# luanfujun/Langevin-MCMC

Measured on AMD Instinct MI355X. Metric: MALA chain-steps/sec, torus scene, higher is better.
Workload: dtype f32

## Files before the change

### langevin-mcmc_amd/csrc/device/kernels.h

```cpp
#pragma once
#include <hip/hip_runtime.h>

#include "dchain.h"
#include "dstep_params.h"

namespace lmcd {
struct H2Arrays;
struct MalaPipe;
struct H2Bins;
struct H2MCParam;
}

void LaunchSeedRng(int n, long long firstSeed, uint64_t *state, uint32_t *tab, hipStream_t s);
void LaunchLowerBoundProbe(int n, const float *cdf, int nq, const float *u, int *out, hipStream_t s);
void LaunchRngProbe(int nSeeds, const unsigned long long *seeds, int mode, int n, float mean, float stddev, uint32_t *tabScratch, uint32_t *out, hipStream_t s);
void LaunchPluginGrad(int c, int l, const float *in, float *out, int wantGrad, hipStream_t s);
void LaunchPluginHess(int c, int l, const float *in, float *stage , float *out, hipStream_t s);
void LaunchCacheProbe(const lmcd::DCache *cache, int dim, int n, const float *u, int *row, const float *query, const int *cl, float *pdf, hipStream_t s);
void LaunchTransProbe(int n, int mode, const float *x, const float *y, float *o, hipStream_t s);
void LaunchStreamProbe(long long nWords, const float *in, float *out, hipStream_t s);
void LaunchAddInto(float *dst, const float *src, size_t n, hipStream_t s);
void LaunchAddIntoF64(double *dst, const double *src, size_t n, hipStream_t s);
void LaunchAddIntoI64(long long *dst, const long long *src, size_t n, hipStream_t s);
void LaunchFilmFixedToFloat(const long long *fx, float *rgb, size_t n, hipStream_t s);
// ... 22 lines not shown
                     uint32_t *tabScratch, float *contribScratch, const uint64_t *seedCkState, const uint32_t *seedCkTicks, float *initPath, float *initContrib,
                     float *initScoreSum, hipStream_t s);
void LaunchDirect(const lmcd::DScene &S, const lmcd::Film &film, int directSpp, int minDepth, int maxDepth, int bvhDepth, bool waveKernel, uint32_t *tabScratch,
                  hipStream_t s);
void LaunchBidirMC(const lmcd::DScene &S, const lmcd::Film &film, int nThreads, int samplesPerThread, uint32_t *tabScratch, float *contribScratch, hipStream_t s);
void LaunchMC(const lmcd::DScene &S, const lmcd::Film &film, bool bidirectional, int spp, int minDepth, int maxDepth, long long streamBegin, long long streamEnd,
              uint32_t *tabScratch, unsigned long long *counters, hipStream_t s);
long long MCThreads(const lmcd::DScene &S, long long streamBegin, long long streamEnd);
void LaunchMCFixedToFloat(const long long *fx, float *rgb, size_t n, int spp, hipStream_t s);
void LaunchSetupChains(const lmcd::ChainArrays &A, int chainBegin, long long perChain, long long chainsNeedExtra, hipStream_t s);
void LaunchFirstKind(const lmcd::DScene &S, const lmcd::DCache *cache, const lmcd::ChainArrays &A, const lmcd::StepParams &P, hipStream_t s);
void LaunchStepLarge(const lmcd::DScene &S, const lmcd::DCache *cache, const lmcd::ChainArrays &A, const lmcd::Film &film, const lmcd::StepParams &P,
                     const int *list, const int *listCount, const lmcd::NextLists &next, float *gradBuf, int gradStride, bool glossy, int gridBlocks, int bvhStackNeed, int blockThreads, hipStream_t s);
void LaunchStepLargeMux(const lmcd::DScene &S, const lmcd::DCache *cache, const lmcd::ChainArrays &A, const lmcd::Film &film, const lmcd::StepParams &P,
                     const int *list, const int *listCount, const lmcd::NextLists &next, float *gradBuf, int gradStride, bool glossy, int gridBlocks, int bvhStackNeed, int blockThreads, hipStream_t s);
void LaunchStepLargeCache(const lmcd::DScene &S, const lmcd::DCache *cache, const lmcd::ChainArrays &A, const lmcd::Film &film, const lmcd::StepParams &P,
                     const int *list, const int *listCount, const lmcd::NextLists &next, float *gradBuf, int gradStride, bool glossy, int gridBlocks, int bvhStackNeed, int blockThreads, hipStream_t s);
void LaunchStepSmallGrad(const lmcd::DScene &S, const lmcd::DCache *cache, const lmcd::ChainArrays &A, const lmcd::Film &film, const lmcd::StepParams &P,
                         const int *list, const int *listCount, const lmcd::NextLists &next, float *gradBuf, int gradStride, bool glossy, int gridBlocks, hipStream_t s);
void LaunchStepSmallLeanGrad(const lmcd::DScene &S, const lmcd::DCache *cache, const lmcd::ChainArrays &A, const lmcd::Film &film, const lmcd::StepParams &P, const int *list,
                             const int *listCount, const lmcd::NextLists &next, float *gradBuf, int gradStride, bool glossy, int gridBlocks, int blockThreads, int bvhStackNeed,
                             hipStream_t s);
void LaunchStepSmallPlain(const lmcd::DScene &S, const lmcd::DCache *cache, const lmcd::ChainArrays &A, const lmcd::Film &film, const lmcd::StepParams &P,
                          const int *list, const int *listCount, const lmcd::NextLists &next, int bvhDepth, bool glossy, int gridBlocks, int blockThreads,
                          bool profile, hipStream_t s);
void LaunchStepResident(const lmcd::DScene &S, const lmcd::DCache *cache, const lmcd::ChainArrays &A, const lmcd::Film &film, const lmcd::StepParams &P, int maxSteps,
                        int lanes, unsigned long long *guard, bool glossy, int mux, int bvhStackNeed, hipStream_t s);
void LaunchH2Begin(const lmcd::DScene &S, const lmcd::ChainArrays &A, const lmcd::StepParams &P, const lmcd::H2Arrays &H, const int *list, const int *listCount, int gridBlocks,
                   hipStream_t s);
void LaunchH2Perturb(const lmcd::DScene &S, const lmcd::ChainArrays &A, const lmcd::StepParams &P, const lmcd::H2Arrays &H, const int *list, const int *listCount,
                     int bvhStackNeed, int gridBlocks, hipStream_t s);
void LaunchH2Finish(const lmcd::DScene &S, const lmcd::DCache *cache, const lmcd::ChainArrays &A, const lmcd::Film &film, const lmcd::StepParams &P, const lmcd::H2Arrays &H,
                    const int *list, const int *listCount, int gridBlocks, hipStream_t s);
void LaunchH2Hess(const float *rec, const lmcd::H2Bins &bins, int N, const float *scene38 , float *hout, int gridBlocks, hipStream_t s);
void LaunchH2Gauss(const lmcd::H2Bins &bins, int N, const float *hout, const lmcd::H2MCParam &param, int expFlags, const int *chainFlags, int stage, float *gaussBuf,
                   const float *offsetSoA, float *px, int gridBlocks, hipStream_t s);
void LaunchH2Sample(const int *list, const int *listCount, int N, const int *chainFlags, const unsigned char *stepKind, const float *curContrib, const float *gaussBuf,
                    float sigma, float *offsetSoA, float *py, int gridBlocks, hipStream_t s);
void LaunchMalaBegin(const lmcd::DScene &S, const lmcd::DCache *cache, const lmcd::ChainArrays &A, const lmcd::StepParams &P, const lmcd::MalaPipe &M, const int *list,
                     const int *listCount, int gridBlocks, hipStream_t s);
void LaunchMalaMid(const lmcd::DScene &S, const lmcd::DCache *cache, const lmcd::ChainArrays &A, const lmcd::StepParams &P, const lmcd::MalaPipe &M, const int *list,
                   const int *listCount, int bvhStackNeed, bool glossy, int gridBlocks, hipStream_t s);
void LaunchMalaFinish(const lmcd::DScene &S, const lmcd::DCache *cache, const lmcd::ChainArrays &A, const lmcd::Film &film, const lmcd::StepParams &P, const lmcd::MalaPipe &M,
                      const int *list, const int *listCount, int gridBlocks, hipStream_t s);
void LaunchMalaGrad(const float *rec, const lmcd::H2Bins &bins, int N, const float *scene38 , float *gout, int gridBlocks, hipStream_t s);
void LaunchHessBatch(int c, int l, int n, const float *primarySoA, const float *scene, const float *vertSoA, float *logLum, float *gradSoA, float *hessSoA,
                     hipStream_t s);
// ... 41 lines not shown
```

### langevin-mcmc_amd/csrc/device/step_kernel.h

```cpp
#pragma once
#include "dstep.h"
#include "kernels.h"

namespace lmcd {

__device__ __forceinline__ void BlockReduceStats(const StepStats &st, unsigned long long *counters, double *weightSum, int *sh) {
    int *sInt = sh;
    float &sW = *reinterpret_cast<float *>(sh + 8);
    __syncthreads();
    if (threadIdx.x == 0) {
        for (int k = 0; k < 8; k++) sInt[k] = 0;
        sW = 0.f;
    }
    __syncthreads();
    int v[8] = {st.steps, st.large, st.accepted, st.gradCalls, st.cacheQueries, st.cacheHits, st.resets, st.lean};
    float w = st.wsum;
    for (int off = 32; off > 0; off >>= 1) {
        for (int k = 0; k < 8; k++) v[k] += __shfl_down(v[k], off);
        w += __shfl_down(w, off);
    }
    if ((threadIdx.x & 63) == 0) {
        for (int k = 0; k < 8; k++)
            if (v[k]) atomicAdd(&sInt[k], v[k]);
        atomicAdd(&sW, w);
    }
    __syncthreads();
    if (threadIdx.x == 0) {
        for (int k = 0; k < 8; k++)
            if (sInt[k]) atomicAdd(&counters[k], (unsigned long long)sInt[k]);
        if (sW != 0.f) atomicAdd(weightSum, (double)sW);
    }
}

#ifndef LMC_STEP_WAVES
#define LMC_STEP_WAVES 2
#endif
#ifndef LMC_STEP_WAVES_GLOSSY_LARGE
#define LMC_STEP_WAVES_GLOSSY_LARGE 3
#endif
template <class FILM, bool WITH_LARGE, bool WITH_SMALL, bool WITH_GRAD, bool GLOSSY, bool LDS_STACK = false, int MUX = 0, bool QUANT = false>
__global__ void __launch_bounds__(256, (GLOSSY && WITH_LARGE && !WITH_SMALL && LDS_STACK) ? LMC_STEP_WAVES_GLOSSY_LARGE : LMC_STEP_WAVES) k_step(DScene S, const DCache *cache, ChainArrays A, FILM film, StepParams P, const int *list, const int *listCount,
                                              NextLists next, float *gradBuf, int gradStride) {
    if ((int)(blockIdx.x * blockDim.x) >= *listCount) return;
    LMC_RNG_JUMP_INIT();
    LMC_MAT_LDS_INIT(S);
    extern __shared__ int ldsStack[];
    StepStats st;
    const int total = *listCount;
    const int tid = blockIdx.x * blockDim.x + threadIdx.x;
    for (int j = tid; j < total; j += gridDim.x * blockDim.x) {
        const int i = list[j];
        Rng rng = LoadChainRng(A, P.chainBegin, S.opt.seedOffset, i);
        GradWork gw{gradBuf, (size_t)gradStride, (size_t)tid};
        const int kind = WITH_LARGE ? KIND_LARGE : KIND_SMALL;
        if constexpr (LDS_STACK) {
            LdsStackT<GLOSSY, QUANT> stk{ldsStack + threadIdx.x, (int)blockDim.x, 0};
            StepChain<WITH_LARGE, WITH_SMALL, WITH_GRAD, MUX>(S, *cache, A, film, P, i, kind, rng, gw, st, stk);
        } else {
            LocalStackT<GLOSSY> stk;
            StepChain<WITH_LARGE, WITH_SMALL, WITH_GRAD, MUX>(S, *cache, A, film, P, i, kind, rng, gw, st, stk);
        }
        QueueNext(S, *cache, A, P, i, rng);
        StoreChainRng(A, i, rng);
    }
    __shared__ int sStats[9];
// ... 5 lines not shown
```

### langevin-mcmc_amd/csrc/device/step_large.hip

```cpp
#ifndef LMC_NO_RNG_JUMP_LDS
#define LMC_RNG_JUMP_LDS
#endif
#include "step_kernel.h"

using namespace lmcd;

template <class FILM>
static void LaunchStepLargeT(const DScene &S, const DCache *cache, const ChainArrays &A, const FILM &film, const StepParams &P, const int *list, const int *listCount,
                     const NextLists &next, float *gradBuf, int gradStride, bool glossy, int gridBlocks, int bvhStackNeed, int blockThreads, hipStream_t s) {
    RequireJumpLdsBlock(blockThreads);
    if (bvhStackNeed <= BVH_LDS_STACK) {
        const int blocks = gridBlocks * (256 / blockThreads);
        const size_t ldsBytes = (size_t)blockThreads * ((bvhStackNeed + 7) / 8 * 8) * sizeof(int);
        const bool quant = S.qnodes != nullptr;
        if (glossy && quant) hipLaunchKernelGGL((k_step<FILM, true, false, false, true, true, 0, true>), dim3(blocks), dim3(blockThreads), ldsBytes, s, S, cache, A, film, P, list, listCount, next, gradBuf, gradStride);
        else if (glossy) hipLaunchKernelGGL((k_step<FILM, true, false, false, true, true>), dim3(blocks), dim3(blockThreads), ldsBytes, s, S, cache, A, film, P, list, listCount, next, gradBuf, gradStride);
        else if (quant) hipLaunchKernelGGL((k_step<FILM, true, false, false, false, true, 0, true>), dim3(blocks), dim3(blockThreads), ldsBytes, s, S, cache, A, film, P, list, listCount, next, gradBuf, gradStride);
        else
            hipLaunchKernelGGL((k_step<FILM, true, false, false, false, true>), dim3(blocks), dim3(blockThreads), ldsBytes, s, S, cache, A, film, P, list, listCount, next, gradBuf, gradStride);
        return;
    }
    if (glossy) hipLaunchKernelGGL((k_step<FILM, true, false, false, true>), dim3(gridBlocks), dim3(256), 0, s, S, cache, A, film, P, list, listCount, next, gradBuf, gradStride);
    else
        hipLaunchKernelGGL((k_step<FILM, true, false, false, false>), dim3(gridBlocks), dim3(256), 0, s, S, cache, A, film, P, list, listCount, next, gradBuf, gradStride);
}
void LaunchStepLarge(const DScene &S, const DCache *cache, const ChainArrays &A, const Film &film, const StepParams &P, const int *list, const int *listCount,
                     const NextLists &next, float *gradBuf, int gradStride, bool glossy, int gridBlocks, int bvhStackNeed, int blockThreads, hipStream_t s) {
    DispatchFilm(film, [&](const auto &f) { LaunchStepLargeT(S, cache, A, f, P, list, listCount, next, gradBuf, gradStride, glossy, gridBlocks, bvhStackNeed, blockThreads, s); });
}
```

### langevin-mcmc_amd/csrc/device/step_large_cache.hip

```cpp
#ifndef LMC_NO_RNG_JUMP_LDS
#define LMC_RNG_JUMP_LDS
#endif
#include "step_kernel.h"

using namespace lmcd;

template <class FILM>
static void LaunchStepLargeCacheT(const DScene &S, const DCache *cache, const ChainArrays &A, const FILM &film, const StepParams &P, const int *list, const int *listCount,
                     const NextLists &next, float *gradBuf, int gradStride, bool glossy, int gridBlocks, int bvhStackNeed, int blockThreads, hipStream_t s) {
    RequireJumpLdsBlock(blockThreads);
    if (bvhStackNeed <= BVH_LDS_STACK) {
        const int blocks = gridBlocks * (256 / blockThreads);
        const size_t ldsBytes = (size_t)blockThreads * ((bvhStackNeed + 7) / 8 * 8) * sizeof(int);
        if (glossy) hipLaunchKernelGGL((k_step<FILM, true, false, false, true, true, 2>), dim3(blocks), dim3(blockThreads), ldsBytes, s, S, cache, A, film, P, list, listCount, next, gradBuf, gradStride);
        else
            hipLaunchKernelGGL((k_step<FILM, true, false, false, false, true, 2>), dim3(blocks), dim3(blockThreads), ldsBytes, s, S, cache, A, film, P, list, listCount, next, gradBuf, gradStride);
        return;
    }
    if (glossy) hipLaunchKernelGGL((k_step<FILM, true, false, false, true, false, 2>), dim3(gridBlocks), dim3(256), 0, s, S, cache, A, film, P, list, listCount, next, gradBuf, gradStride);
    else
        hipLaunchKernelGGL((k_step<FILM, true, false, false, false, false, 2>), dim3(gridBlocks), dim3(256), 0, s, S, cache, A, film, P, list, listCount, next, gradBuf, gradStride);
}
void LaunchStepLargeCache(const DScene &S, const DCache *cache, const ChainArrays &A, const Film &film, const StepParams &P, const int *list, const int *listCount,
                     const NextLists &next, float *gradBuf, int gradStride, bool glossy, int gridBlocks, int bvhStackNeed, int blockThreads, hipStream_t s) {
    DispatchFilm(film, [&](const auto &f) { LaunchStepLargeCacheT(S, cache, A, f, P, list, listCount, next, gradBuf, gradStride, glossy, gridBlocks, bvhStackNeed, blockThreads, s); });
}

__global__ void k_cache_probe(const DCache *cache, int dim, int n, const float *u, int *row, const float *query, const int *cl, float *pdf) {
    const DCacheDim &D = cache->d[dim];
    for (int i = blockIdx.x * blockDim.x + threadIdx.x; i < n; i += gridDim.x * blockDim.x) {
        row[i] = CacheSampleRow(D, u[i]);
        float q[MAXPSS];
        for (int k = 0; k < dim; k++) q[k] = query[(size_t)i * dim + k];
        pdf[i] = EvalPdfCache(D, dim, q, cl[2 * i], cl[2 * i + 1]);
    }
}
void LaunchCacheProbe(const DCache *cache, int dim, int n, const float *u, int *row, const float *query, const int *cl, float *pdf, hipStream_t s) {
    hipLaunchKernelGGL(k_cache_probe, dim3((n + 63) / 64), dim3(64), 0, s, cache, dim, n, u, row, query, cl, pdf);
}
```

### langevin-mcmc_amd/csrc/device/step_large_mux.hip

```cpp
#ifndef LMC_NO_RNG_JUMP_LDS
#define LMC_RNG_JUMP_LDS
#endif
#include "step_kernel.h"

using namespace lmcd;

template <class FILM>
static void LaunchStepLargeMuxT(const DScene &S, const DCache *cache, const ChainArrays &A, const FILM &film, const StepParams &P, const int *list, const int *listCount,
                     const NextLists &next, float *gradBuf, int gradStride, bool glossy, int gridBlocks, int bvhStackNeed, int blockThreads, hipStream_t s) {
    RequireJumpLdsBlock(blockThreads);
    if (bvhStackNeed <= BVH_LDS_STACK) {
        const int blocks = gridBlocks * (256 / blockThreads);
        const size_t ldsBytes = (size_t)blockThreads * ((bvhStackNeed + 7) / 8 * 8) * sizeof(int);
        if (glossy) hipLaunchKernelGGL((k_step<FILM, true, false, false, true, true, 1>), dim3(blocks), dim3(blockThreads), ldsBytes, s, S, cache, A, film, P, list, listCount, next, gradBuf, gradStride);
        else
            hipLaunchKernelGGL((k_step<FILM, true, false, false, false, true, 1>), dim3(blocks), dim3(blockThreads), ldsBytes, s, S, cache, A, film, P, list, listCount, next, gradBuf, gradStride);
        return;
    }
    if (glossy) hipLaunchKernelGGL((k_step<FILM, true, false, false, true, false, 1>), dim3(gridBlocks), dim3(256), 0, s, S, cache, A, film, P, list, listCount, next, gradBuf, gradStride);
    else
        hipLaunchKernelGGL((k_step<FILM, true, false, false, false, false, 1>), dim3(gridBlocks), dim3(256), 0, s, S, cache, A, film, P, list, listCount, next, gradBuf, gradStride);
}
void LaunchStepLargeMux(const DScene &S, const DCache *cache, const ChainArrays &A, const Film &film, const StepParams &P, const int *list, const int *listCount,
                     const NextLists &next, float *gradBuf, int gradStride, bool glossy, int gridBlocks, int bvhStackNeed, int blockThreads, hipStream_t s) {
    DispatchFilm(film, [&](const auto &f) { LaunchStepLargeMuxT(S, cache, A, f, P, list, listCount, next, gradBuf, gradStride, glossy, gridBlocks, bvhStackNeed, blockThreads, s); });
}
```

### langevin-mcmc_amd/csrc/device/step_small_grad.hip

```cpp
#include "step_kernel.h"

using namespace lmcd;

template <class FILM>
static void LaunchStepSmallGradT(const DScene &S, const DCache *cache, const ChainArrays &A, const FILM &film, const StepParams &P, const int *list, const int *listCount,
                         const NextLists &next, float *gradBuf, int gradStride, bool glossy, int gridBlocks, hipStream_t s) {
    (void)glossy;
    hipLaunchKernelGGL((k_step<FILM, false, true, true, true>), dim3(gridBlocks), dim3(256), 0, s, S, cache, A, film, P, list, listCount, next, gradBuf, gradStride);
}
void LaunchStepSmallGrad(const DScene &S, const DCache *cache, const ChainArrays &A, const Film &film, const StepParams &P, const int *list, const int *listCount,
                         const NextLists &next, float *gradBuf, int gradStride, bool glossy, int gridBlocks, hipStream_t s) {
    DispatchFilm(film, [&](const auto &f) { LaunchStepSmallGradT(S, cache, A, f, P, list, listCount, next, gradBuf, gradStride, glossy, gridBlocks, s); });
}
```

### langevin-mcmc_amd/csrc/device/step_small_plain.hip

```cpp
#include <cstdlib>
#include <type_traits>

#ifndef LMC_NO_RNG_JUMP_LDS
#define LMC_RNG_JUMP_LDS
#endif
#include "dsmall.h"
#include "step_kernel.h"

using namespace lmcd;

template <class FILM, bool USE_LDS_STACK, bool GLOSSY, bool PROF = false, bool LIGHTLESS = false, bool QUANT = false>
#ifndef LMC_LEAN_K
#define LMC_LEAN_K 1
#endif
#ifndef LMC_LEAN_WAVES
#define LMC_LEAN_WAVES 2
#endif
#ifndef LMC_LEAN_WAVES_GLOSSY_LIGHTLESS
#define LMC_LEAN_WAVES_GLOSSY_LIGHTLESS 3
#endif
__global__ void __launch_bounds__(256, (GLOSSY && LIGHTLESS) ? LMC_LEAN_WAVES_GLOSSY_LIGHTLESS : LMC_LEAN_WAVES) k_step_small(DScene S, const DCache *cache, ChainArrays A, FILM film, StepParams P, const int *list,
                                                    const int *listCount, NextLists next, int stackWords) {
    extern __shared__ float lds[];
    if ((int)(blockIdx.x * blockDim.x) >= *listCount) return;
    LMC_RNG_JUMP_INIT();
    LMC_MAT_LDS_INIT(S);
    StepStats st;
    const int total = *listCount;
    const int tid = blockIdx.x * blockDim.x + threadIdx.x;
    const LdsView L{lds + threadIdx.x, (int)blockDim.x, stackWords};
    typename std::conditional<PROF, WaveProf, NoProf>::type prof;
    if constexpr (PROF) prof.Start();
    for (int j = tid; j < total; j += gridDim.x * blockDim.x) {
        const int i = list[j];
        Rng rng = LoadChainRng(A, P.chainBegin, S.opt.seedOffset, i);
#if LMC_LEAN_K > 1
#pragma unroll 1
        for (int rep = 0;; rep++) {
#endif
        if (USE_LDS_STACK) {
            LdsStackT<GLOSSY, QUANT> stk{reinterpret_cast<int *>(L.base), L.stride, 0};
            SmallStepLean<false, LIGHTLESS>(S, *cache, A, film, P, i, rng, L, stk, st, prof);
        } else {
            LocalStackT<GLOSSY, QUANT> stk;
            SmallStepLean<false, LIGHTLESS>(S, *cache, A, film, P, i, rng, L, stk, st, prof);
        }
        const unsigned char nk = QueueNext(S, *cache, A, P, i, rng);
#if LMC_LEAN_K > 1
            if (rep + 1 >= LMC_LEAN_K || (nk & 3) != NEXT_SMALL_PLAIN) break;
        }
#else
        (void)nk;
#endif
        StoreChainRng(A, i, rng);
        prof.Mark(PR_QUEUE);
    }
    if constexpr (PROF) {
        if ((threadIdx.x & 63) == 0) {
            for (int r = 0; r < PR_COUNT; r++) atomicAdd(&A.prof[r], prof.acc[r]);
            atomicAdd(&A.prof[PR_COUNT], 1ull);
        }
    }
    if (!LMC_EXP(P.expFlags, 8)) BlockReduceStats(st, A.counters, A.weightSum, reinterpret_cast<int *>(lds));
}

template <class FILM>
static void LaunchStepSmallPlainT(const DScene &S, const DCache *cache, const ChainArrays &A, const FILM &film, const StepParams &P, const int *list, const int *listCount,
                          const NextLists &next, int bvhDepth, bool glossy, int gridBlocks, int blockThreads, bool profile, hipStream_t s) {
    RequireJumpLdsBlock(blockThreads);
    const int stackWords = LeanStackWords(bvhDepth);
    size_t ldsBytes = (size_t)blockThreads * LeanLdsWordsPerThread(stackWords) * sizeof(float);
    if (const char *e = getenv("LMC_EXP_LDS_EXTRA")) ldsBytes += (size_t)atoi(e);
    const bool lds = bvhDepth <= BVH_LDS_STACK;
#define LMC_LAUNCH_SMALL(...) hipLaunchKernelGGL((k_step_small<FILM, __VA_ARGS__>), dim3(gridBlocks), dim3(blockThreads), ldsBytes, s, S, cache, A, film, P, list, listCount, next, stackWords)
    const bool quant = S.qnodes != nullptr && lds && !profile;
    if (profile && lds && glossy) LMC_LAUNCH_SMALL(true, true, true);
    else if (profile && lds && !glossy) LMC_LAUNCH_SMALL(true, false, true);
    else if (lds && !glossy && S.opt.leanLightless) {
        if (quant) LMC_LAUNCH_SMALL(true, false, false, true, true);
        else
            LMC_LAUNCH_SMALL(true, false, false, true);
    } else if (lds && glossy && S.opt.leanLightless) {
        if (quant) LMC_LAUNCH_SMALL(true, true, false, true, true);
        else
            LMC_LAUNCH_SMALL(true, true, false, true);
    } else if (lds && !glossy) {
        if (quant) LMC_LAUNCH_SMALL(true, false, false, false, true);
        else
            LMC_LAUNCH_SMALL(true, false);
    } else if (lds && glossy) {
        if (quant) LMC_LAUNCH_SMALL(true, true, false, false, true);
        else
            LMC_LAUNCH_SMALL(true, true);
    } else if (!glossy)
        LMC_LAUNCH_SMALL(false, false);
    else
        LMC_LAUNCH_SMALL(false, true);
#undef LMC_LAUNCH_SMALL
}
void LaunchStepSmallPlain(const DScene &S, const DCache *cache, const ChainArrays &A, const Film &film, const StepParams &P, const int *list, const int *listCount,
                          const NextLists &next, int bvhDepth, bool glossy, int gridBlocks, int blockThreads, bool profile, hipStream_t s) {
    DispatchFilm(film, [&](const auto &f) { LaunchStepSmallPlainT(S, cache, A, f, P, list, listCount, next, bvhDepth, glossy, gridBlocks, blockThreads, profile, s); });
}
```

### langevin-mcmc_amd/csrc/host/context.cpp

```cpp
#include <hip/hip_runtime.h>
#include <dlfcn.h>

#include <algorithm>
#include <chrono>
#include <condition_variable>
#include <mutex>
#include <cstdio>
#include <cstdlib>
#include <cstring>
#include <exception>
#include <functional>
#include <memory>
#include <stdexcept>
#include <string>
#include <thread>
#include <vector>

#include <rccl/rccl.h>

#include "../../../include/lmc_abi.h"
#include "../device/drng.h"
#include "../device/kernels.h"
#include "../device/upload.h"
#include "../device/dh2coop.h"
// ... 65 lines not shown
    DevBuf<KdNode> nodes;
    DevBuf<uint2> gridWords;
    DevBuf<int> gridCellStart;
    DevBuf<unsigned short> gridIdx;
    int gridG = 0, gridM = 0;
    int gridCoord[4] = {0, 1, 2, 3};
    DevBuf<int> vind;
    bool ready = false;
    bool relevant = false;
};

}

static int GetRcclDestroy(void *comm);

struct lmc_ctx {
    std::unique_ptr<lmc::Scene> scene;
    int device = 0;
    int useGradient = 1;
    int maxDervDepth = 8;
    bool useOccFilter = true;
    int gridDims = 4;
    bool largeLdsStack = true;
    int largeBlock = 64;
    bool leanGrad = true;
    bool anyDeepCache = false;
    bool sortH2mc = true;
    bool sortGeneric = true;
    DevBuf<int> listScratch, listScratch2, sortBins, sortBins2;
    int expFlags = 0;
    hipStream_t stream = nullptr;
    hipStream_t sideStream[2] = {nullptr, nullptr};
    static constexpr int H2_MAX_PARTS = 4;
    hipStream_t partStream[H2_MAX_PARTS - 1] = {};
    hipEvent_t partFork = nullptr, partJoin[H2_MAX_PARTS - 1] = {};
    hipEvent_t h2HeadDone[H2_MAX_PARTS] = {};
    int h2HeadParts = 0;
    hipEvent_t forkEvent = nullptr, joinEvent[2] = {nullptr, nullptr};
    hipEvent_t packedEvent = nullptr, copiedEvent = nullptr;
    DevBuf<float> filmStage;
    DevBuf<long long> filmStageFx;
    DevBuf<double> weightStage;
    hipEvent_t filmReadyEvent = nullptr, sliceReducedEvent = nullptr, weightsCopiedEvent = nullptr;
    int groupPeerPairs = 0, groupPeerEnabled = 0, groupDevices = 0;
    double hostIssueMs = 0;
    long long hostIssueSteps = 0;
// ... 39 lines not shown
    DevBuf<uint64_t> rngState;
    DevBuf<uint32_t> rngTab;
    DevBuf<unsigned char> rngTicked;
    DevBuf<float> curPath, pathBuf1, curContrib, scoreSum, gaussian, gaussian1, curSplat, chV1, chV2, chCurrNewV2, chPropNewV1, chPropNewV2, chPss, chLastPss, chPath, chContrib, pathWeight,
        lastScoreSum, lastScore, contribList, pushData, initPath, initContrib, initScoreSum, initLsAll;
    DevBuf<unsigned char> initCLAll;
    DevBuf<unsigned char> nextKind;
    DevBuf<int> flags, curSplatCount, adjacentReject, sampleIdx, numSamples, pushDim;
    DevBuf<unsigned long long> counters, prof;
    bool profileLean = false;
    DevBuf<double> weightSum;
    DevBuf<float> gradBuf;
    DevBuf<float> h2Rec, h2Out, h2Gauss, h2Offset, h2Py, h2Px, h2PropContrib;
    DevBuf<int> h2Step, h2Items, h2BinOf, h2Counts, h2SubList, h2SubCount;
    H2Bins h2Bins[H2_MAX_PARTS][2] = {};
    int h2Parts = 1, h2PartStride = 0;
    const int *h2SplitOf = nullptr;
    DevBuf<unsigned char> h2Kind;
    H2Arrays H2{};
    int h2HessGrid = 0, h2GaussGrid = 0;
    bool malaPipe = true;
    MalaPipe MP{};
    int gradStride = 0, stepGrid = 0;
    int leanBlock = 64, leanGrid = 0, sortPlain = 0;
    bool relocate = false;
    DevBuf<int> chainId, slotOf, relocTileCount, relocTileHist, relocMembers, relocSorted, relocCount;
    DevBuf<unsigned> relocPlacedKey;
    DevBuf<unsigned char> stepKind;
    bool relocFine = false;
    DevBuf<float> relocStaging;
    RelocBuffers RB{};
    long long relocations = 0;
    int pendingResort = 0;
    int resortEvery = 0, resortFirst = 0;
    int resortEveryOpt = -1, resortFirstOpt = -1;
    long long stepsSinceInit = 0, resorts = 0;
    DevBuf<unsigned> sortKeys[2];
    DevBuf<int> sortVals[2], sortHist, sortScanSums;
    RelocSortBuffers RS{};
    DevBuf<int> lists[2][3], listCounts[2];
    int parity = 0;
    CacheDimHost cacheDims[PSS_MAX_LENGTH + 1];
    DCache cacheHost;
    DevBuf<DCache> cacheDev;
    DevBuf<int> cacheCounts;
    DevBuf<unsigned long long> pushTiles;
    DevBuf<int> gridScratchStart, gridScratchCursor, gridScratchWordCount, gridTileSums;
// ... 287 lines not shown
        int lo = 0, hi = 0;
        HIP_CHECK(hipDeviceGetStreamPriorityRange(&lo, &hi));
        const char *e = getenv("LMC_STREAM_PRIO");
        const int mode = e ? atoi(e) : 1;
        const char *eL = getenv("LMC_STREAM_PRIO_LARGE");
        const int modeL = eL ? atoi(eL) : mode;
        for (int k = 0; k < 2; k++) {
            const int m = k == 0 ? modeL : mode;
            HIP_CHECK(hipStreamCreateWithPriority(&c->sideStream[k], hipStreamNonBlocking, m > 0 ? hi : m < 0 ? lo : 0));
        }
        for (auto &ps : c->partStream) HIP_CHECK(hipStreamCreateWithPriority(&ps, hipStreamNonBlocking, mode > 0 ? hi : mode < 0 ? lo : 0));
        HIP_CHECK(hipStreamCreateWithPriority(&c->cacheStream, hipStreamNonBlocking, mode > 0 ? hi : mode < 0 ? lo : 0));
        HIP_CHECK(hipHostMalloc((void **)&c->cachePinned, sizeof(DCache), hipHostMallocDefault));
    }
    HIP_CHECK(hipEventCreateWithFlags(&c->partFork, hipEventDisableTiming));
    for (auto &e : c->partJoin) HIP_CHECK(hipEventCreateWithFlags(&e, hipEventDisableTiming));
    HIP_CHECK(hipEventCreateWithFlags(&c->forkEvent, hipEventDisableTiming));
    for (auto &e : c->joinEvent) HIP_CHECK(hipEventCreateWithFlags(&e, hipEventDisableTiming));
    HIP_CHECK(hipEventCreateWithFlags(&c->packedEvent, hipEventDisableTiming));
    HIP_CHECK(hipEventCreateWithFlags(&c->copiedEvent, hipEventDisableTiming));
    if (const char *e = getenv("LMC_OVERLAP")) c->overlap = atoi(e) != 0;
    if (const char *e = getenv("LMC_OCC_FILTER")) c->useOccFilter = atoi(e) != 0;
    if (const char *e = getenv("LMC_LARGE_LDS")) c->largeLdsStack = atoi(e) != 0;
    if (const char *e = getenv("LMC_LARGE_BLOCK")) c->largeBlock = atoi(e) == 64 ? 64 : atoi(e) == 128 ? 128 : 256;
    if (const char *e = getenv("LMC_PROF")) c->profileLean = atoi(e) != 0;
    if (const char *e = getenv("LMC_LEAN_GRAD")) c->leanGrad = atoi(e) != 0;
    if (const char *e = getenv("LMC_MALA_PIPE")) c->malaPipe = atoi(e) != 0;
    if (const char *e = getenv("LMC_EARLY_APPLY")) c->earlyApply = atoi(e) != 0;
    if (const char *e = getenv("LMC_SORT_H2MC")) c->sortH2mc = atoi(e) != 0;
    if (const char *e = getenv("LMC_SORT_GENERIC")) c->sortGeneric = atoi(e) != 0;
    if (const char *e = getenv("LMC_GRID_DIMS")) c->gridDims = std::min(4, std::max(3, atoi(e)));
    if (const char *e = getenv("LMC_FILM_EXACT")) c->filmExact = atoi(e) != 0;
    if (const char *e = getenv("LMC_EXP_OUTLIER_TEST")) c->expFlags |= atoi(e) ? 128 : 0;
    {
        static const struct {
            const char *name;
            int one, two;
        } sw[] = {{"LMC_EXP_NOSPLAT", 1, 1}, {"LMC_EXP_NOQUERY", 2, 2}, {"LMC_EXP_QUERY_STOP", 256, 512}, {"LMC_EXP_NOGRAD", 4, 4}, {"LMC_EXP_NOSTATS", 8, 8},
                  {"LMC_EXP_NOHESS", 16, 16}, {"LMC_EXP_NOEIGEN", 32, 32}, {"LMC_EXP_NOHESSLAUNCH", 64, 64}, {"LMC_EXP_NOTRAV", 1024, 1024}, {"LMC_EXP_NOSTORE", 2048, 2048}, {"LMC_EXP_NOREUSE", 4096, 4096}};
        for (const auto &w : sw) {
            const char *e = getenv(w.name);
            if (!e || atoi(e) == 0) continue;
#ifdef LMC_EXP_SWITCHES
            c->expFlags |= atoi(e) == 2 ? w.two : w.one;
#else
            throw std::runtime_error(std::string(w.name) + " is set, but this build of liblmc_hip.so has no work-skipping measurement switches (they exist in -DLMC_EXP_SWITCHES builds only: scripts/build_exp.sh, selected with LMC_LIB)");
// ... 521 lines not shown
        if (const char *e = getenv("LMC_RELOC_FINE")) c->relocFine = atoi(e) != 0;
        if (c->resortEvery > 0 || c->relocFine) {
            const size_t nb = RelocSortBlocks((int)N);
            for (int k = 0; k < 2; k++) c->sortKeys[k].Alloc(N, false), c->sortVals[k].Alloc(N, false);
            c->sortHist.Alloc(256 * nb, false), c->sortScanSums.Alloc(256 * nb / 2048 + 2, false);
            c->RS = RelocSortBuffers{{c->sortKeys[0].p, c->sortKeys[1].p}, {c->sortVals[0].p, c->sortVals[1].p}, c->sortHist.p, c->sortScanSums.p};
        }
        c->RB = RelocBuffers{c->relocPlacedKey.p, c->relocTileCount.p, c->relocTileHist.p, c->relocMembers.p, c->relocSorted.p, c->relocCount.p, c->relocStaging.p, (int)N, c->relocFine};
        A.chainId = c->chainId.p, A.slotOf = c->slotOf.p, A.stepKind = c->stepKind.p;
    } else {
        A.chainId = nullptr, A.slotOf = nullptr, A.stepKind = nullptr;
        for (auto *b : {&c->chainId, &c->slotOf, &c->relocTileCount, &c->relocTileHist, &c->relocMembers, &c->relocSorted, &c->relocCount}) b->Free();
        c->relocPlacedKey.Free(), c->stepKind.Free(), c->relocStaging.Free();
    }
    if (!U.fromCheckpoint) {
        LaunchSeedRng((int)N, (long long)chainBegin + c->S.opt.seedOffset, c->rngState.p, c->rngTab.p, s);
        LaunchSetupChains(A, chainBegin, perChain, chainsNeedExtra, s);
    }
    c->stepGrid = (int)std::min<size_t>((N + 255) / 256, 4096);
    c->gradStride = c->stepGrid * 256;
    if (const char *e = getenv("LMC_LEAN_BLOCK")) c->leanBlock = std::max(64, std::min(256, atoi(e) / 64 * 64));
    c->sortPlain = c->S.glossy ? 4 : 0;
    if (const char *e = getenv("LMC_SORT_PLAIN")) c->sortPlain = atoi(e);
    c->leanGrid = (int)std::min<size_t>((N + c->leanBlock - 1) / c->leanBlock, (size_t)4096 * 256 / c->leanBlock);
    c->gradBuf.Alloc(c->useGradient ? (size_t)c->gradStride * 640 : 1, false);
    size_t maxGridCells = 0;
    for (int d = 0; d <= PSS_MAX_LENGTH; d++) {
        CacheDimHost &cd = c->cacheDims[d];
        cd.ready = false;
        cd.relevant = (d % 2 == 0) && d >= 2 * std::max(c->S.opt.minDepth, 3) && d <= 2 * c->S.opt.maxDepth;
        if (cd.relevant) {
            cd.pss.Alloc((size_t)PSS_MAX_SIZE * d), cd.v1.Alloc((size_t)PSS_MAX_SIZE * d), cd.v2.Alloc((size_t)PSS_MAX_SIZE * d);
            cd.weight.Alloc(PSS_MAX_SIZE);
            if (sampleCache) cd.extra.Alloc((size_t)PSS_MAX_SIZE * CACHE_ROW_EXTRA), cd.distCdf.Alloc(PSS_MAX_SIZE + 1);
            cd.gridG = CacheGridG(d), cd.gridM = std::min(c->gridDims, d);
            size_t cells = 1, nbrs = 1;
            for (int k = 0; k < cd.gridM; k++) cells *= cd.gridG, nbrs *= 3;
            cd.gridWords.Alloc((cells + 31) / 32, false), cd.gridCellStart.Alloc(std::min(cells, (size_t)PSS_MAX_SIZE * nbrs) + 1, false), cd.gridIdx.Alloc((size_t)PSS_MAX_SIZE * nbrs, false);
            maxGridCells = std::max(maxGridCells, cells);
            cd.nodes.Alloc(KD_MAX_NODES, false), cd.vind.Alloc(PSS_MAX_SIZE, false);
            const int sl = (d - 6) / 2;
            if (sl >= 0 && sl < CACHE_SLOTS && d == 6 + 2 * sl) {
                if (!c->rowsPinned[sl]) HIP_CHECK(hipHostMalloc(reinterpret_cast<void **>(&c->rowsPinned[sl]), (size_t)PSS_MAX_SIZE * PSS_MAX_LENGTH * sizeof(float)));
                if (!c->treePinned[sl]) HIP_CHECK(hipHostMalloc(reinterpret_cast<void **>(&c->treePinned[sl]), (size_t)KD_MAX_NODES * sizeof(KdNode) + (size_t)PSS_MAX_SIZE * sizeof(int)));
            }
        }
    }
// ... 588 lines not shown
        }
        if (c->relocate) {
            if (c->relocations == 2 && c->RB.capacity == (int)c->N && c->N >= 65536 && c->resortEvery == 0 && !getenv("LMC_RELOC_STAGING_FULL")) {
                static std::mutex stagingMutex;
                std::lock_guard<std::mutex> lock(stagingMutex);
                HIP_CHECK(hipStreamSynchronize(sL));
                const size_t cap = c->N / 2;
                c->RB.staging = nullptr, c->RB.capacity = 0;
                c->relocStaging.Alloc(cap * RelocRecordWords(c->S.opt.maxDepth), false);
                c->RB.staging = c->relocStaging.p, c->RB.capacity = (int)cap;
            }
            if (c->relocFine) LaunchRelocateFine(c->A, c->S.opt.maxDepth, c->RB, c->RS, c->S.opt.h2mc != 0, sL);
            else
                LaunchRelocate(c->A, c->S.opt.maxDepth, c->RB, c->S.opt.h2mc != 0, sL);
            c->relocations++;
        }
    };
    if (!genericFirst) large();
    if (c->timing) HIP_CHECK(hipEventRecord(ev.e[6], sG));
    LaunchGeneric(c, film, P, cur, cnt, next, sG);
    if (c->timing) HIP_CHECK(hipEventRecord(ev.e[7], sG));
    if (genericFirst) large();
    if (c->timing) HIP_CHECK(hipEventRecord(ev.e[1], s));
    if (!c->S.opt.h2mc) LaunchStepSmallPlain(c->S, c->cacheDev.p, c->A, film, P, c->lists[cur][2].p, cnt + 2, next, c->bvhDepth, c->S.glossy != 0, c->leanGrid, c->leanBlock, c->profileLean, s);
    if (c->timing) HIP_CHECK(hipEventRecord(ev.e[2], s));
    if (c->overlap) {
        HIP_CHECK(hipEventRecord(c->joinEvent[0], sL));
        HIP_CHECK(hipStreamWaitEvent(s, c->joinEvent[0], 0));
        if (c->needGeneric) {
            HIP_CHECK(hipEventRecord(c->joinEvent[1], sG));
            HIP_CHECK(hipStreamWaitEvent(s, c->joinEvent[1], 0));
        }
    }
    return exchange;
}
void DebugResort(lmc_ctx *c) {
    hipStream_t s = c->stream;
    const int mode = c->pendingResort;
    c->pendingResort = 0;
    const size_t N = c->N;
    HIP_CHECK(hipStreamSynchronize(s));
    if (c->RB.capacity < (int)N) {
        c->relocStaging.Alloc(N * RelocRecordWords(c->S.opt.maxDepth), false);
        c->RB.staging = c->relocStaging.p, c->RB.capacity = (int)N;
    }
    DevBuf<unsigned long long> keys;
    keys.Alloc(N, false);
// ... 57 lines not shown
    }
    if (c->needGeneric && c->S.opt.h2mc && c->overlap && c->h2Parts >= 2) {
        LaunchSplitList(c->lists[nxt][1].p, c->listCounts[nxt].p + 1, c->h2Parts, c->h2SubList.p, c->h2PartStride, c->h2SubCount.p, c->stepGrid * 4 + 1, s);
        c->h2SplitOf = c->lists[nxt][1].p;
    }
}
}
}
static void WarmStepLaunches(lmc_ctx *c) {
    if (getenv("LMC_NO_WARM_LAUNCH")) return;
    const Film film = StepFilm(c);
    const StepParams P = MakeStepParams(c);
    c->warmCounts.Alloc(4);
    NextLists next{c->lists[1][0].p, c->lists[1][1].p, c->lists[1][2].p, c->listCounts[1].p};
    hipStream_t s = c->stream, sL = c->overlap ? c->sideStream[0] : s, sG = c->overlap ? c->sideStream[1] : s;
    const int *cnt = c->warmCounts.p;
    LaunchLarge(c, film, P, 0, cnt, next, sL);
    LaunchGeneric(c, film, P, 0, cnt, next, sG);
    if (c->MP.rec && !c->allCachesReady) {
        c->allCachesReady = true;
        LaunchGeneric(c, film, P, 0, cnt, next, sG);
        c->allCachesReady = false;
    }
    LaunchStepSmallPlain(c->S, c->cacheDev.p, c->A, film, P, c->lists[0][2].p, cnt + 2, next, c->bvhDepth, c->S.glossy != 0, c->leanGrid, c->leanBlock, c->profileLean, s);
    HIP_CHECK(hipStreamSynchronize(sL));
    HIP_CHECK(hipStreamSynchronize(sG));
    HIP_CHECK(hipStreamSynchronize(s));
}
extern "C++" {
namespace {
constexpr long long kResidentBudget = 1ll << 21;
constexpr int kResidentMaxK = 32;
int ResidentLanes(const lmc_ctx *c) { return c->residentLanes ? c->residentLanes : c->N <= 65536 ? 32 : 64; }
int ResidentK(const lmc_ctx *c) {
    if (c->residentSteps <= 0 || c->N <= 0) return 0;
    const long long byBudget = std::max(1ll, kResidentBudget / (long long)c->N);
    return (int)std::min<long long>({(long long)c->residentSteps, (long long)kResidentMaxK, byBudget});
}
bool ResidentEligible(lmc_ctx *c) {
    if (c->residentSteps <= 0 || c->S.opt.h2mc) return false;
    return c->allCachesReady || !CachePending(c);
}
void RunResident(lmc_ctx *c, int steps) {
    HIP_CHECK(hipSetDevice(c->device));
    hipStream_t s = c->stream;
    c->filmReduced = false;
    const int K = ResidentK(c);
// ... 1956 lines not shown
```

Before: 687.2 million.

## Pack step kernel args into a struct read via kernarg pointer; one-item lean grid

Step kernels now take a single StepKernArgs struct and read their fields by reference through the kernarg segment pointer, rather than copying large by-value structs into registers. The lean small-step kernel drops its grid-stride loop and launches one thread per chain, with the grid sized from the chain count instead of a capped grid. A new occupancy bound is added for the lambertian quantized large kernel, and an env toggle can disable the lean LDS stack. The aim is to cut register pressure and argument copy cost and to avoid loop overhead, at the price of launching more blocks when N is large.

```diff
diff --git a/langevin-mcmc_amd/csrc/device/kernels.h b/langevin-mcmc_amd/csrc/device/kernels.h
--- a/langevin-mcmc_amd/csrc/device/kernels.h
+++ b/langevin-mcmc_amd/csrc/device/kernels.h
@@ -68,7 +68,7 @@
                              const int *listCount, const lmcd::NextLists &next, float *gradBuf, int gradStride, bool glossy, int gridBlocks, int blockThreads, int bvhStackNeed,
                              hipStream_t s);
 void LaunchStepSmallPlain(const lmcd::DScene &S, const lmcd::DCache *cache, const lmcd::ChainArrays &A, const lmcd::Film &film, const lmcd::StepParams &P,
-                          const int *list, const int *listCount, const lmcd::NextLists &next, int bvhDepth, bool glossy, int gridBlocks, int blockThreads,
+                          const int *list, const int *listCount, const lmcd::NextLists &next, int bvhDepth, bool glossy, bool ldsStack, int blockThreads,
                           bool profile, hipStream_t s);
 void LaunchStepResident(const lmcd::DScene &S, const lmcd::DCache *cache, const lmcd::ChainArrays &A, const lmcd::Film &film, const lmcd::StepParams &P, int maxSteps,
                         int lanes, unsigned long long *guard, bool glossy, int mux, int bvhStackNeed, hipStream_t s);
diff --git a/langevin-mcmc_amd/csrc/device/step_kernel.h b/langevin-mcmc_amd/csrc/device/step_kernel.h
--- a/langevin-mcmc_amd/csrc/device/step_kernel.h
+++ b/langevin-mcmc_amd/csrc/device/step_kernel.h
@@ -38,9 +38,43 @@
 #ifndef LMC_STEP_WAVES_GLOSSY_LARGE
 #define LMC_STEP_WAVES_GLOSSY_LARGE 3
 #endif
+#ifndef LMC_STEP_WAVES_LAMBERTIAN_LARGE
+#define LMC_STEP_WAVES_LAMBERTIAN_LARGE 3
+#endif
+template <class FILM>
+struct StepKernArgs {
+    DScene S;
+    const DCache *cache;
+    ChainArrays A;
+    FILM film;
+    StepParams P;
+    const int *list, *listCount;
+    float *gradBuf;
+    int gradStride;
+    int stackWords;
+};
+template <class ARGS>
+__device__ __forceinline__ const ARGS &KernArgs() {
+    return *(const ARGS *)__builtin_amdgcn_kernarg_segment_ptr();
+}
+template <class ARGS>
+inline void LaunchKernArgs(void (*kernel)(ARGS), dim3 grid, dim3 block, size_t ldsBytes, hipStream_t s, const ARGS &K) {
+    hipLaunchKernelGGL(kernel, grid, block, ldsBytes, s, K);
+}
 template <class FILM, bool WITH_LARGE, bool WITH_SMALL, bool WITH_GRAD, bool GLOSSY, bool LDS_STACK = false, int MUX = 0, bool QUANT = false>
-__global__ void __launch_bounds__(256, (GLOSSY && WITH_LARGE && !WITH_SMALL && LDS_STACK) ? LMC_STEP_WAVES_GLOSSY_LARGE : LMC_STEP_WAVES) k_step(DScene S, const DCache *cache, ChainArrays A, FILM film, StepParams P, const int *list, const int *listCount,
-                                              NextLists next, float *gradBuf, int gradStride) {
+__global__ void __launch_bounds__(256, !(WITH_LARGE && !WITH_SMALL && LDS_STACK) ? LMC_STEP_WAVES
+                                       : GLOSSY                                ? LMC_STEP_WAVES_GLOSSY_LARGE
+                                       : (MUX == 0 && QUANT)                   ? LMC_STEP_WAVES_LAMBERTIAN_LARGE
+                                                                               : LMC_STEP_WAVES) k_step(StepKernArgs<FILM> ) {
+    const StepKernArgs<FILM> &K = KernArgs<StepKernArgs<FILM>>();
+    const DScene &S = K.S;
+    const DCache *cache = K.cache;
+    const ChainArrays &A = K.A;
+    const FILM &film = K.film;
+    const StepParams &P = K.P;
+    const int *list = K.list, *listCount = K.listCount;
+    float *gradBuf = K.gradBuf;
+    const int gradStride = K.gradStride;
     if ((int)(blockIdx.x * blockDim.x) >= *listCount) return;
     LMC_RNG_JUMP_INIT();
     LMC_MAT_LDS_INIT(S);
diff --git a/langevin-mcmc_amd/csrc/device/step_large.hip b/langevin-mcmc_amd/csrc/device/step_large.hip
--- a/langevin-mcmc_amd/csrc/device/step_large.hip
+++ b/langevin-mcmc_amd/csrc/device/step_large.hip
@@ -9,20 +9,21 @@
 static void LaunchStepLargeT(const DScene &S, const DCache *cache, const ChainArrays &A, const FILM &film, const StepParams &P, const int *list, const int *listCount,
                      const NextLists &next, float *gradBuf, int gradStride, bool glossy, int gridBlocks, int bvhStackNeed, int blockThreads, hipStream_t s) {
     RequireJumpLdsBlock(blockThreads);
+    const StepKernArgs<FILM> K{S, cache, A, film, P, list, listCount, gradBuf, gradStride, 0};
     if (bvhStackNeed <= BVH_LDS_STACK) {
         const int blocks = gridBlocks * (256 / blockThreads);
         const size_t ldsBytes = (size_t)blockThreads * ((bvhStackNeed + 7) / 8 * 8) * sizeof(int);
         const bool quant = S.qnodes != nullptr;
-        if (glossy && quant) hipLaunchKernelGGL((k_step<FILM, true, false, false, true, true, 0, true>), dim3(blocks), dim3(blockThreads), ldsBytes, s, S, cache, A, film, P, list, listCount, next, gradBuf, gradStride);
-        else if (glossy) hipLaunchKernelGGL((k_step<FILM, true, false, false, true, true>), dim3(blocks), dim3(blockThreads), ldsBytes, s, S, cache, A, film, P, list, listCount, next, gradBuf, gradStride);
-        else if (quant) hipLaunchKernelGGL((k_step<FILM, true, false, false, false, true, 0, true>), dim3(blocks), dim3(blockThreads), ldsBytes, s, S, cache, A, film, P, list, listCount, next, gradBuf, gradStride);
+        if (glossy && quant) LaunchKernArgs(k_step<FILM, true, false, false, true, true, 0, true>, dim3(blocks), dim3(blockThreads), ldsBytes, s, K);
+        else if (glossy) LaunchKernArgs(k_step<FILM, true, false, false, true, true>, dim3(blocks), dim3(blockThreads), ldsBytes, s, K);
+        else if (quant) LaunchKernArgs(k_step<FILM, true, false, false, false, true, 0, true>, dim3(blocks), dim3(blockThreads), ldsBytes, s, K);
         else
-            hipLaunchKernelGGL((k_step<FILM, true, false, false, false, true>), dim3(blocks), dim3(blockThreads), ldsBytes, s, S, cache, A, film, P, list, listCount, next, gradBuf, gradStride);
+            LaunchKernArgs(k_step<FILM, true, false, false, false, true>, dim3(blocks), dim3(blockThreads), ldsBytes, s, K);
         return;
     }
-    if (glossy) hipLaunchKernelGGL((k_step<FILM, true, false, false, true>), dim3(gridBlocks), dim3(256), 0, s, S, cache, A, film, P, list, listCount, next, gradBuf, gradStride);
+    if (glossy) LaunchKernArgs(k_step<FILM, true, false, false, true>, dim3(gridBlocks), dim3(256), 0, s, K);
     else
-        hipLaunchKernelGGL((k_step<FILM, true, false, false, false>), dim3(gridBlocks), dim3(256), 0, s, S, cache, A, film, P, list, listCount, next, gradBuf, gradStride);
+        LaunchKernArgs(k_step<FILM, true, false, false, false>, dim3(gridBlocks), dim3(256), 0, s, K);
 }
 void LaunchStepLarge(const DScene &S, const DCache *cache, const ChainArrays &A, const Film &film, const StepParams &P, const int *list, const int *listCount,
                      const NextLists &next, float *gradBuf, int gradStride, bool glossy, int gridBlocks, int bvhStackNeed, int blockThreads, hipStream_t s) {
diff --git a/langevin-mcmc_amd/csrc/device/step_large_cache.hip b/langevin-mcmc_amd/csrc/device/step_large_cache.hip
--- a/langevin-mcmc_amd/csrc/device/step_large_cache.hip
+++ b/langevin-mcmc_amd/csrc/device/step_large_cache.hip
@@ -9,17 +9,18 @@
 static void LaunchStepLargeCacheT(const DScene &S, const DCache *cache, const ChainArrays &A, const FILM &film, const StepParams &P, const int *list, const int *listCount,
                      const NextLists &next, float *gradBuf, int gradStride, bool glossy, int gridBlocks, int bvhStackNeed, int blockThreads, hipStream_t s) {
     RequireJumpLdsBlock(blockThreads);
+    const StepKernArgs<FILM> K{S, cache, A, film, P, list, listCount, gradBuf, gradStride, 0};
     if (bvhStackNeed <= BVH_LDS_STACK) {
         const int blocks = gridBlocks * (256 / blockThreads);
         const size_t ldsBytes = (size_t)blockThreads * ((bvhStackNeed + 7) / 8 * 8) * sizeof(int);
-        if (glossy) hipLaunchKernelGGL((k_step<FILM, true, false, false, true, true, 2>), dim3(blocks), dim3(blockThreads), ldsBytes, s, S, cache, A, film, P, list, listCount, next, gradBuf, gradStride);
+        if (glossy) LaunchKernArgs(k_step<FILM, true, false, false, true, true, 2>, dim3(blocks), dim3(blockThreads), ldsBytes, s, K);
         else
-            hipLaunchKernelGGL((k_step<FILM, true, false, false, false, true, 2>), dim3(blocks), dim3(blockThreads), ldsBytes, s, S, cache, A, film, P, list, listCount, next, gradBuf, gradStride);
+            LaunchKernArgs(k_step<FILM, true, false, false, false, true, 2>, dim3(blocks), dim3(blockThreads), ldsBytes, s, K);
         return;
     }
-    if (glossy) hipLaunchKernelGGL((k_step<FILM, true, false, false, true, false, 2>), dim3(gridBlocks), dim3(256), 0, s, S, cache, A, film, P, list, listCount, next, gradBuf, gradStride);
+    if (glossy) LaunchKernArgs(k_step<FILM, true, false, false, true, false, 2>, dim3(gridBlocks), dim3(256), 0, s, K);
     else
-        hipLaunchKernelGGL((k_step<FILM, true, false, false, false, false, 2>), dim3(gridBlocks), dim3(256), 0, s, S, cache, A, film, P, list, listCount, next, gradBuf, gradStride);
+        LaunchKernArgs(k_step<FILM, true, false, false, false, false, 2>, dim3(gridBlocks), dim3(256), 0, s, K);
 }
 void LaunchStepLargeCache(const DScene &S, const DCache *cache, const ChainArrays &A, const Film &film, const StepParams &P, const int *list, const int *listCount,
                      const NextLists &next, float *gradBuf, int gradStride, bool glossy, int gridBlocks, int bvhStackNeed, int blockThreads, hipStream_t s) {
diff --git a/langevin-mcmc_amd/csrc/device/step_large_mux.hip b/langevin-mcmc_amd/csrc/device/step_large_mux.hip
--- a/langevin-mcmc_amd/csrc/device/step_large_mux.hip
+++ b/langevin-mcmc_amd/csrc/device/step_large_mux.hip
@@ -9,17 +9,18 @@
 static void LaunchStepLargeMuxT(const DScene &S, const DCache *cache, const ChainArrays &A, const FILM &film, const StepParams &P, const int *list, const int *listCount,
                      const NextLists &next, float *gradBuf, int gradStride, bool glossy, int gridBlocks, int bvhStackNeed, int blockThreads, hipStream_t s) {
     RequireJumpLdsBlock(blockThreads);
+    const StepKernArgs<FILM> K{S, cache, A, film, P, list, listCount, gradBuf, gradStride, 0};
     if (bvhStackNeed <= BVH_LDS_STACK) {
         const int blocks = gridBlocks * (256 / blockThreads);
         const size_t ldsBytes = (size_t)blockThreads * ((bvhStackNeed + 7) / 8 * 8) * sizeof(int);
-        if (glossy) hipLaunchKernelGGL((k_step<FILM, true, false, false, true, true, 1>), dim3(blocks), dim3(blockThreads), ldsBytes, s, S, cache, A, film, P, list, listCount, next, gradBuf, gradStride);
+        if (glossy) LaunchKernArgs(k_step<FILM, true, false, false, true, true, 1>, dim3(blocks), dim3(blockThreads), ldsBytes, s, K);
         else
-            hipLaunchKernelGGL((k_step<FILM, true, false, false, false, true, 1>), dim3(blocks), dim3(blockThreads), ldsBytes, s, S, cache, A, film, P, list, listCount, next, gradBuf, gradStride);
+            LaunchKernArgs(k_step<FILM, true, false, false, false, true, 1>, dim3(blocks), dim3(blockThreads), ldsBytes, s, K);
         return;
     }
-    if (glossy) hipLaunchKernelGGL((k_step<FILM, true, false, false, true, false, 1>), dim3(gridBlocks), dim3(256), 0, s, S, cache, A, film, P, list, listCount, next, gradBuf, gradStride);
+    if (glossy) LaunchKernArgs(k_step<FILM, true, false, false, true, false, 1>, dim3(gridBlocks), dim3(256), 0, s, K);
     else
-        hipLaunchKernelGGL((k_step<FILM, true, false, false, false, false, 1>), dim3(gridBlocks), dim3(256), 0, s, S, cache, A, film, P, list, listCount, next, gradBuf, gradStride);
+        LaunchKernArgs(k_step<FILM, true, false, false, false, false, 1>, dim3(gridBlocks), dim3(256), 0, s, K);
 }
 void LaunchStepLargeMux(const DScene &S, const DCache *cache, const ChainArrays &A, const Film &film, const StepParams &P, const int *list, const int *listCount,
                      const NextLists &next, float *gradBuf, int gradStride, bool glossy, int gridBlocks, int bvhStackNeed, int blockThreads, hipStream_t s) {
diff --git a/langevin-mcmc_amd/csrc/device/step_small_grad.hip b/langevin-mcmc_amd/csrc/device/step_small_grad.hip
--- a/langevin-mcmc_amd/csrc/device/step_small_grad.hip
+++ b/langevin-mcmc_amd/csrc/device/step_small_grad.hip
@@ -6,7 +6,8 @@
 static void LaunchStepSmallGradT(const DScene &S, const DCache *cache, const ChainArrays &A, const FILM &film, const StepParams &P, const int *list, const int *listCount,
                          const NextLists &next, float *gradBuf, int gradStride, bool glossy, int gridBlocks, hipStream_t s) {
     (void)glossy;
-    hipLaunchKernelGGL((k_step<FILM, false, true, true, true>), dim3(gridBlocks), dim3(256), 0, s, S, cache, A, film, P, list, listCount, next, gradBuf, gradStride);
+    const StepKernArgs<FILM> K{S, cache, A, film, P, list, listCount, gradBuf, gradStride, 0};
+    LaunchKernArgs(k_step<FILM, false, true, true, true>, dim3(gridBlocks), dim3(256), 0, s, K);
 }
 void LaunchStepSmallGrad(const DScene &S, const DCache *cache, const ChainArrays &A, const Film &film, const StepParams &P, const int *list, const int *listCount,
                          const NextLists &next, float *gradBuf, int gradStride, bool glossy, int gridBlocks, hipStream_t s) {
diff --git a/langevin-mcmc_amd/csrc/device/step_small_plain.hip b/langevin-mcmc_amd/csrc/device/step_small_plain.hip
--- a/langevin-mcmc_amd/csrc/device/step_small_plain.hip
+++ b/langevin-mcmc_amd/csrc/device/step_small_plain.hip
@@ -19,9 +19,16 @@
 #ifndef LMC_LEAN_WAVES_GLOSSY_LIGHTLESS
 #define LMC_LEAN_WAVES_GLOSSY_LIGHTLESS 3
 #endif
-__global__ void __launch_bounds__(256, (GLOSSY && LIGHTLESS) ? LMC_LEAN_WAVES_GLOSSY_LIGHTLESS : LMC_LEAN_WAVES) k_step_small(DScene S, const DCache *cache, ChainArrays A, FILM film, StepParams P, const int *list,
-                                                    const int *listCount, NextLists next, int stackWords) {
+__global__ void __launch_bounds__(256, (GLOSSY && LIGHTLESS) ? LMC_LEAN_WAVES_GLOSSY_LIGHTLESS : LMC_LEAN_WAVES) k_step_small(StepKernArgs<FILM> ) {
     extern __shared__ float lds[];
+    const StepKernArgs<FILM> &K = KernArgs<StepKernArgs<FILM>>();
+    const DScene &S = K.S;
+    const DCache *cache = K.cache;
+    const ChainArrays &A = K.A;
+    const FILM &film = K.film;
+    const StepParams &P = K.P;
+    const int *list = K.list, *listCount = K.listCount;
+    const int stackWords = K.stackWords;
     if ((int)(blockIdx.x * blockDim.x) >= *listCount) return;
     LMC_RNG_JUMP_INIT();
     LMC_MAT_LDS_INIT(S);
@@ -31,7 +38,7 @@
     const LdsView L{lds + threadIdx.x, (int)blockDim.x, stackWords};
     typename std::conditional<PROF, WaveProf, NoProf>::type prof;
     if constexpr (PROF) prof.Start();
-    for (int j = tid; j < total; j += gridDim.x * blockDim.x) {
+    if (const int j = tid; j < total) {
         const int i = list[j];
         Rng rng = LoadChainRng(A, P.chainBegin, S.opt.seedOffset, i);
 #if LMC_LEAN_K > 1
@@ -66,13 +73,15 @@
 
 template <class FILM>
 static void LaunchStepSmallPlainT(const DScene &S, const DCache *cache, const ChainArrays &A, const FILM &film, const StepParams &P, const int *list, const int *listCount,
-                          const NextLists &next, int bvhDepth, bool glossy, int gridBlocks, int blockThreads, bool profile, hipStream_t s) {
+                          const NextLists &next, int bvhDepth, bool glossy, bool ldsStack, int blockThreads, bool profile, hipStream_t s) {
     RequireJumpLdsBlock(blockThreads);
+    const int gridBlocks = (A.N + blockThreads - 1) / blockThreads;
     const int stackWords = LeanStackWords(bvhDepth);
     size_t ldsBytes = (size_t)blockThreads * LeanLdsWordsPerThread(stackWords) * sizeof(float);
     if (const char *e = getenv("LMC_EXP_LDS_EXTRA")) ldsBytes += (size_t)atoi(e);
-    const bool lds = bvhDepth <= BVH_LDS_STACK;
-#define LMC_LAUNCH_SMALL(...) hipLaunchKernelGGL((k_step_small<FILM, __VA_ARGS__>), dim3(gridBlocks), dim3(blockThreads), ldsBytes, s, S, cache, A, film, P, list, listCount, next, stackWords)
+    const bool lds = ldsStack && bvhDepth <= BVH_LDS_STACK;
+    const StepKernArgs<FILM> K{S, cache, A, film, P, list, listCount, nullptr, 0, stackWords};
+#define LMC_LAUNCH_SMALL(...) LaunchKernArgs(k_step_small<FILM, __VA_ARGS__>, dim3(gridBlocks), dim3(blockThreads), ldsBytes, s, K)
     const bool quant = S.qnodes != nullptr && lds && !profile;
     if (profile && lds && glossy) LMC_LAUNCH_SMALL(true, true, true);
     else if (profile && lds && !glossy) LMC_LAUNCH_SMALL(true, false, true);
@@ -99,6 +108,6 @@
 #undef LMC_LAUNCH_SMALL
 }
 void LaunchStepSmallPlain(const DScene &S, const DCache *cache, const ChainArrays &A, const Film &film, const StepParams &P, const int *list, const int *listCount,
-                          const NextLists &next, int bvhDepth, bool glossy, int gridBlocks, int blockThreads, bool profile, hipStream_t s) {
-    DispatchFilm(film, [&](const auto &f) { LaunchStepSmallPlainT(S, cache, A, f, P, list, listCount, next, bvhDepth, glossy, gridBlocks, blockThreads, profile, s); });
+                          const NextLists &next, int bvhDepth, bool glossy, bool ldsStack, int blockThreads, bool profile, hipStream_t s) {
+    DispatchFilm(film, [&](const auto &f) { LaunchStepSmallPlainT(S, cache, A, f, P, list, listCount, next, bvhDepth, glossy, ldsStack, blockThreads, profile, s); });
 }
diff --git a/langevin-mcmc_amd/csrc/host/context.cpp b/langevin-mcmc_amd/csrc/host/context.cpp
--- a/langevin-mcmc_amd/csrc/host/context.cpp
+++ b/langevin-mcmc_amd/csrc/host/context.cpp
@@ -111,6 +111,7 @@
     bool useOccFilter = true;
     int gridDims = 4;
     bool largeLdsStack = true;
+    bool leanLdsStack = true;
     int largeBlock = 64;
     bool leanGrad = true;
     bool anyDeepCache = false;
@@ -196,7 +197,7 @@
     bool malaPipe = true;
     MalaPipe MP{};
     int gradStride = 0, stepGrid = 0;
-    int leanBlock = 64, leanGrid = 0, sortPlain = 0;
+    int leanBlock = 64, sortPlain = 0;
     bool relocate = false;
     DevBuf<int> chainId, slotOf, relocTileCount, relocTileHist, relocMembers, relocSorted, relocCount;
     DevBuf<unsigned> relocPlacedKey;
@@ -530,6 +531,7 @@
     if (const char *e = getenv("LMC_OVERLAP")) c->overlap = atoi(e) != 0;
     if (const char *e = getenv("LMC_OCC_FILTER")) c->useOccFilter = atoi(e) != 0;
     if (const char *e = getenv("LMC_LARGE_LDS")) c->largeLdsStack = atoi(e) != 0;
+    if (const char *e = getenv("LMC_LEAN_LDS")) c->leanLdsStack = atoi(e) != 0;
     if (const char *e = getenv("LMC_LARGE_BLOCK")) c->largeBlock = atoi(e) == 64 ? 64 : atoi(e) == 128 ? 128 : 256;
     if (const char *e = getenv("LMC_PROF")) c->profileLean = atoi(e) != 0;
     if (const char *e = getenv("LMC_LEAN_GRAD")) c->leanGrad = atoi(e) != 0;
@@ -1097,7 +1099,6 @@
     if (const char *e = getenv("LMC_LEAN_BLOCK")) c->leanBlock = std::max(64, std::min(256, atoi(e) / 64 * 64));
     c->sortPlain = c->S.glossy ? 4 : 0;
     if (const char *e = getenv("LMC_SORT_PLAIN")) c->sortPlain = atoi(e);
-    c->leanGrid = (int)std::min<size_t>((N + c->leanBlock - 1) / c->leanBlock, (size_t)4096 * 256 / c->leanBlock);
     c->gradBuf.Alloc(c->useGradient ? (size_t)c->gradStride * 640 : 1, false);
     size_t maxGridCells = 0;
     for (int d = 0; d <= PSS_MAX_LENGTH; d++) {
@@ -1732,7 +1733,7 @@
     if (c->timing) HIP_CHECK(hipEventRecord(ev.e[7], sG));
     if (genericFirst) large();
     if (c->timing) HIP_CHECK(hipEventRecord(ev.e[1], s));
-    if (!c->S.opt.h2mc) LaunchStepSmallPlain(c->S, c->cacheDev.p, c->A, film, P, c->lists[cur][2].p, cnt + 2, next, c->bvhDepth, c->S.glossy != 0, c->leanGrid, c->leanBlock, c->profileLean, s);
+    if (!c->S.opt.h2mc) LaunchStepSmallPlain(c->S, c->cacheDev.p, c->A, film, P, c->lists[cur][2].p, cnt + 2, next, c->bvhDepth, c->S.glossy != 0, c->leanLdsStack, c->leanBlock, c->profileLean, s);
     if (c->timing) HIP_CHECK(hipEventRecord(ev.e[2], s));
     if (c->overlap) {
         HIP_CHECK(hipEventRecord(c->joinEvent[0], sL));
@@ -1836,7 +1837,7 @@
         LaunchGeneric(c, film, P, 0, cnt, next, sG);
         c->allCachesReady = false;
     }
-    LaunchStepSmallPlain(c->S, c->cacheDev.p, c->A, film, P, c->lists[0][2].p, cnt + 2, next, c->bvhDepth, c->S.glossy != 0, c->leanGrid, c->leanBlock, c->profileLean, s);
+    LaunchStepSmallPlain(c->S, c->cacheDev.p, c->A, film, P, c->lists[0][2].p, cnt + 2, next, c->bvhDepth, c->S.glossy != 0, c->leanLdsStack, c->leanBlock, c->profileLean, s);
     HIP_CHECK(hipStreamSynchronize(sL));
     HIP_CHECK(hipStreamSynchronize(sG));
     HIP_CHECK(hipStreamSynchronize(s));
```

Result: faster. 722.8 million, median of 6 (+5.2%).
